# orhosko/tiny-ntt

Measured on AMD Instinct MI355X. Metric: negacyclic poly-mults/sec (n=4096, 60-bit q), bit-exact vs cg_ntt.py, higher is better.
Workload: dtype u64; 1 GPU; n=4096, q=2^60-2^14+1 (60-bit), global batch 65536 = 65536 rows on this GPU, LCG-seeded rows resident in HBM (BASELINE configs[2]); n=4096, q=1152921504606830593, rows_per_gpu=65536, global_batch=65536, variant=fused, kernel=polymul_fused_kernel, lazy_reduction=True, lib_build_id=05922c9b9694243b, parallelism=batch-sharded x1, no data-path collective

## Files before the change

### __graft_entry__.py

```python
import ctypes
import os
import subprocess
import sys

ROOT = os.path.dirname(os.path.abspath(__file__))
REFERENCE = os.environ.get("TINY_NTT_REFERENCE", "/root/reference")


def _make(directory, *targets):
    cmd = ["make", f"-j{min(8, os.cpu_count() or 1)}", "-C", os.path.join(ROOT, directory), *targets]
    r = subprocess.run(cmd, stdout=subprocess.PIPE, stderr=subprocess.STDOUT, text=True)
    if r.returncode != 0:
        sys.stderr.write(r.stdout)
        raise RuntimeError(f"build failed: {' '.join(cmd)}")


def build() -> None:
    _make("tiny_ntt_amd/csrc")
    _make("oracle", "all")
    _make("tests/emu")
    _make("tests/emu", "-f", "Makefile.prepared")
    _make("tests/emu", "-f", "Makefile.dot")
    _make("tests/devprobe")
    if os.path.isdir(os.path.join(REFERENCE, "software_benchmark")):
        _make("oracle", "ref", f"REFERENCE={REFERENCE}")
    sys.path.insert(0, ROOT)
    import tiny_ntt_amd
    from tiny_ntt_amd import engine
    lib = engine.load_library()
    missing = [s for s in engine.EXPORTED_SYMBOLS if not hasattr(lib, s)]
    if missing:
        raise RuntimeError(f"libtinyntt.so lacks symbols: {missing}")


def smoke() -> None:
    sys.path.insert(0, ROOT)
    import numpy as np
    from tiny_ntt_amd import engine

    n, q, psi = 4096, 1152921504606830593, 431606828070683274
    plan = engine.Plan(n, q, psi, device=0)
    rng = np.random.default_rng(7)
    batch = 4
    a = rng.integers(0, q, size=(batch, n), dtype=np.uint64)
    b = rng.integers(0, q, size=(batch, n), dtype=np.uint64)
    a[0, :] = q - 1
    c = plan.poly_mult(a, b)
    c_cg = plan.poly_mult(a, b, variant="cg8")

    so = os.path.join(ROOT, "oracle", "_build", "liboracle.so")
    if not os.path.exists(so):
        _make("oracle", "all")
    orc = ctypes.CDLL(so)
    P = ctypes.POINTER(ctypes.c_uint64)
    orc.tn_oracle_nwc_poly_mult_batch.argtypes = [P, P, P, ctypes.c_size_t, ctypes.c_size_t, ctypes.c_uint64, ctypes.c_uint64]
    ref = np.empty_like(a)
    rc = orc.tn_oracle_nwc_poly_mult_batch(a.ctypes.data_as(P), b.ctypes.data_as(P), ref.ctypes.data_as(P), batch, n, q, psi)
    assert rc == 0
    assert np.array_equal(c, ref), "fused kernel differs from the oracle"
    assert np.array_equal(c_cg, ref), "cg8 kernel differs from the oracle"
    print(f"smoke ok: n={n} q={q} batch={batch} fused(lazy={plan.is_lazy}) and cg8 bit-exact vs oracle")


if __name__ == "__main__":
    build()
    if len(sys.argv) > 1 and sys.argv[1] == "smoke":
        smoke()
```

### tiny_ntt_amd/csrc/fused_core.h

```cpp
#pragma once
#include <type_traits>
#include "modarith.h"

#ifndef TN_ABL_UNIFORM_TW
#define TN_ABL_UNIFORM_TW 0
#endif

namespace tn {

template <int B, int E_, typename F> struct StaticFor {
  TN_HD static void run(F& f) { f(std::integral_constant<int, B>()); StaticFor<B + 1, E_, F>::run(f); }
};
template <int E_, typename F> struct StaticFor<E_, E_, F> { TN_HD static void run(F&) {} };
template <int B, int E_, typename F> TN_HD void static_for(F&& f) { StaticFor<B, E_, F>::run(f); }

#ifndef TN_FUSED_LPT10
#define TN_FUSED_LPT10 3
#endif
#ifndef TN_FUSED_LPT12
#define TN_FUSED_LPT12 3
#endif
constexpr int fused_lpt(int logn) {
  return logn == 8 ? 2 : logn == 9 ? 3 : logn == 10 ? TN_FUSED_LPT10 : logn == 11 ? 3 : logn == 12 ? TN_FUSED_LPT12 : logn == 13 ? 3 : 0;
}
// ... 221 lines not shown
    d.pw_fold_b = d.fout > PW_IN;
    for (int r = 0; r < R; r += 2) {
      if (!BC) { b[r] = b[r + 1] = PW_OUT; continue; }
      long a0 = b[r], a1 = b[r + 1];
      if (a0 > BC_AMAX) { d.bcfold[r] = true; a0 = FOLDED; }
      if (a1 > BC_AMAX) { d.bcfold[r + 1] = true; a1 = FOLDED; }
      b[r] = tmax(a0) + tmax(tmax(a1));
      b[r + 1] = tmax(a0) + tmax(a1);
    }
    for (int g = BC ? 1 : 0; g < LOGN; ++g) {
      const int s = LOGN - 1 - g;
      if (g > 0 && phase_of(s) != phase_of(s + 1)) {
        long m = 0;
        for (int r = 0; r < R; ++r) m = b[r] > m ? b[r] : m;
        for (int r = 0; r < R; ++r) b[r] = m;
      }
      const int bit = 1 << bpos_of(s);
      for (int r = 0; r < R; ++r) {
        if (r & bit) continue;
        const int v = r | bit;
        for (int it = 0; it < 2; ++it) {
          if (b[r] + ki(b[v]) * U <= CAP && b[r] + b[v] <= CAP) break;
          if (b[r] >= b[v]) { d.ifold[g][r] = true; b[r] = FOLDED; }
          else { d.ifold[g][v] = true; b[v] = FOLDED; }
        }
        const int Kv = ki(b[v]);
        d.ik[g][r] = (unsigned char)Kv;
        const long bd = b[r] + Kv * U;
        b[r] = b[r] + b[v];
        b[v] = tmax(bd);
      }
    }
    return d;
  }
  static constexpr Data D = build();
};

template <typename Pol, typename Cfg, bool BC = false> struct SchedOf {
  typedef Sched<Pol, Cfg::LOGN> S;
  static constexpr bool fwd_fold(int s, int r) { return S::fwd_fold(s) && !(r & (1 << SplitSched<Cfg>::bpos_of(s))); }
  static constexpr int fwd_k(int, int) { return Pol::TMUL; }
  static constexpr bool inv_fold(int g, int) { return S::inv_fold(g); }
  static constexpr int inv_k(int g, int) { return S::inv_bnd(g); }
  static constexpr bool pw_fold_b() { return false; }
  static constexpr bool pw_ok() { return !Pol::lazy || S::fwd_out() <= Pol::LIMIT - 2; }
};
template <typename Cfg, bool CIN, bool BC> struct SchedOf<Policy<u64, true, CIN>, Cfg, BC> {
  typedef SplitSched<Cfg, CIN, BC> S;
  static constexpr bool fwd_fold(int s, int r) { return S::D.ffold[s][r]; }
  static constexpr int fwd_k(int s, int r) { return S::D.fk[s][r]; }
  static constexpr bool inv_fold(int g, int r) { return S::D.ifold[g][r]; }
  static constexpr int inv_k(int g, int r) { return S::D.ik[g][r]; }
  static constexpr bool pw_fold_b() { return S::D.pw_fold_b; }
  static constexpr bool pw_ok() { return true; }
  static constexpr bool bc_fold(int r) { return S::D.bcfold[r]; }
};

template <typename E> struct TwRefs {
  typedef typename TwOf<E>::type Tw;
  const Tw* __restrict__ glob;
  const Tw* lds;
  Tw* pre;
  const Tw* mid = nullptr;
  u32 zero = 0;
};

template <typename E, typename Cfg, int PH, int S_>
TN_HD typename TwOf<E>::type tw_get(const TwRefs<E>& t, u32 thi, int g) {
  constexpr int bpos = (Cfg::LOGN - 1 - S_) - Cfg::pos(PH);
  if (Cfg::tw_src(PH) == Cfg::TW_REGS) return t.pre[Cfg::pre_off(S_) + g];
  const u32 idx = (1u << S_) + (TN_ABL_UNIFORM_TW ? 0u : (thi << (Cfg::LPT - bpos - 1))) + (u32)g;
  if (Cfg::tw_src(PH) == Cfg::TW_LDS) {
    if (t.mid) return t.mid[(1 << (S_ - Cfg::stage_begin(PH))) - 1 + g];
    return t.lds[idx - Cfg::lds_tw_lo()];
  }
  if (Cfg::tw_src(PH) == Cfg::TW_VEC && t.mid) return t.mid[(1 << (S_ - Cfg::stage_begin(PH))) - 1 + g];
  return t.glob[idx + t.zero];
}

template <typename E, typename Cfg, int PH>
TN_HD void tw_fetch_vec(typename TwOf<E>::type (&mid)[Cfg::R], u32 tau, const typename TwOf<E>::type* __restrict__ glob) {
  const u32 thi = Cfg::thi(PH, tau);
  static_for<Cfg::stage_begin(PH), Cfg::stage_end(PH)>([&](auto s_) {
    constexpr int s = decltype(s_)::value;
    constexpr int bpos = (Cfg::LOGN - 1 - s) - Cfg::pos(PH);
    constexpr int cnt = Cfg::R >> (bpos + 1), off = (1 << (s - Cfg::stage_begin(PH))) - 1;
    const u32 boff = ((1u << s) + (thi << (Cfg::LPT - bpos - 1))) * (u32)sizeof(typename TwOf<E>::type);
    const typename TwOf<E>::type* base = reinterpret_cast<const typename TwOf<E>::type*>(reinterpret_cast<const char*>(glob) + boff);
#pragma unroll
    for (int g = 0; g < cnt; ++g) mid[off + g] = base[g];
  });
}

template <typename E, typename Cfg, int PH>
TN_HD void tw_fetch_mid(typename TwOf<E>::type (&mid)[Cfg::R], u32 tau, const typename TwOf<E>::type* lds_tw) {
  const u32 thi = Cfg::thi(PH, tau);
  static_for<Cfg::stage_begin(PH), Cfg::stage_end(PH)>([&](auto s_) {
    constexpr int s = decltype(s_)::value;
    constexpr int bpos = (Cfg::LOGN - 1 - s) - Cfg::pos(PH);
    constexpr int cnt = Cfg::R >> (bpos + 1), off = (1 << (s - Cfg::stage_begin(PH))) - 1;
#pragma unroll
    for (int g = 0; g < cnt; ++g)
      mid[off + g] = lds_tw[(1u << s) + (thi << (Cfg::LPT - bpos - 1)) + (u32)g - Cfg::lds_tw_lo()];
  });
}

template <typename E, typename Cfg, int S0, int S1>
TN_HD void tw_prefetch_stages(typename TwOf<E>::type* pre, u32 tau, const typename TwOf<E>::type* __restrict__ glob) {
  constexpr int PH = Cfg::PHASES - 1;
  if (Cfg::tw_src(PH) != Cfg::TW_REGS) return;
  const u32 thi = Cfg::thi(PH, tau);
  static_for<S0, S1>([&](auto s_) {
    constexpr int s = decltype(s_)::value;
    constexpr int bpos = (Cfg::LOGN - 1 - s) - Cfg::pos(PH);
    const u32 off = ((1u << s) + (thi << (Cfg::LPT - bpos - 1))) * (u32)sizeof(typename TwOf<E>::type);
    const typename TwOf<E>::type* base = reinterpret_cast<const typename TwOf<E>::type*>(reinterpret_cast<const char*>(glob) + off);
#pragma unroll
    for (int g = 0; g < Cfg::pre_count(s); ++g) pre[Cfg::pre_off(s) + g] = base[g];
  });
}
template <typename E, typename Cfg>
TN_HD void tw_prefetch_raw(typename TwOf<E>::type* pre, u32 tau, const typename TwOf<E>::type* __restrict__ glob) {
  tw_prefetch_stages<E, Cfg, Cfg::stage_begin(Cfg::PHASES - 1), Cfg::LOGN>(pre, tau, glob);
}

template <typename E, typename Cfg>
TN_HD void tw_prefetch(typename TwOf<E>::type (&pre)[Cfg::NPRE], u32 tau, const typename TwOf<E>::type* __restrict__ glob) {
  tw_prefetch_raw<E, Cfg>(pre, tau, glob);
}

template <typename E, typename Cfg, typename Pol, int PH, bool BC = false>
TN_HD void fwd_phase(E (&x)[Cfg::R], u32 tau, const TwRefs<E>& tw, const Arith<E>& ar) {
  typedef SchedOf<Pol, Cfg, BC> SO;
  typedef typename TwOf<E>::type Tw;
  const u32 thi = Cfg::thi(PH, tau);
  constexpr int SEND = BC && Cfg::stage_end(PH) == Cfg::LOGN ? Cfg::LOGN - 1 : Cfg::stage_end(PH);
  static_for<Cfg::stage_begin(PH), SEND>([&](auto s_) {
    constexpr int s = decltype(s_)::value;
    constexpr int bpos = (Cfg::LOGN - 1 - s) - Cfg::pos(PH);
    static_for<0, Cfg::R>([&](auto r_) {
      constexpr int r = decltype(r_)::value;
      if constexpr (Pol::lazy && SO::fwd_fold(s, r)) x[r] = fold(x[r], ar.k, ar.fold_c);
    });
    static_for<0, Cfg::R>([&](auto r_) {
      constexpr int r = decltype(r_)::value;
      if constexpr (!(r & (1 << bpos))) {
        const Tw w = tw_get<E, Cfg, PH, s>(tw, thi, r >> (bpos + 1));
        Pol::template ct<SO::fwd_k(s, r)>(x[r], x[r | (1 << bpos)], w, ar);
      }
    });
  });
}

template <typename E, typename Cfg, typename Pol, int PH, bool BC = false>
TN_HD void inv_phase(E (&x)[Cfg::R], u32 tau, const TwRefs<E>& tw, const Arith<E>& ar) {
  typedef SchedOf<Pol, Cfg, BC> SO;
  typedef typename TwOf<E>::type Tw;
  const u32 thi = Cfg::thi(PH, tau);
  constexpr int SEND = BC && Cfg::stage_end(PH) == Cfg::LOGN ? Cfg::LOGN - 1 : Cfg::stage_end(PH);
  static_for<0, SEND - Cfg::stage_begin(PH)>([&](auto i_) {
    constexpr int s = SEND - 1 - decltype(i_)::value;
    constexpr int g = Cfg::LOGN - 1 - s;
    constexpr int bpos = (Cfg::LOGN - 1 - s) - Cfg::pos(PH);
    static_for<0, Cfg::R>([&](auto r_) {
      constexpr int r = decltype(r_)::value;
      if constexpr (Pol::lazy && SO::inv_fold(g, r)) x[r] = fold(x[r], ar.k, ar.fold_c);
    });
    static_for<0, Cfg::R>([&](auto r_) {
      constexpr int r = decltype(r_)::value;
      if constexpr (!(r & (1 << bpos))) {
        constexpr int BND = SO::inv_k(g, r);
        if constexpr (s == 0) Pol::template gs_last<BND>(x[r], x[r | (1 << bpos)], ar);
        else {
          const Tw w = tw_get<E, Cfg, PH, s>(tw, thi, r >> (bpos + 1));
          Pol::template gs<BND>(x[r], x[r | (1 << bpos)], w, ar);
        }
      }
    });
  });
}

template <typename E, typename Cfg, typename Pol>
TN_HD void load_reduce(E (&x)[Cfg::R], const Arith<E>& ar) {
#pragma unroll
  for (int r = 0; r < Cfg::R / 2; ++r) x[r] = Pol::load(x[r], ar);
}

template <typename E, typename Cfg, int EX, int PH>
TN_HD void ex_store(const E (&x)[Cfg::R], u32 tau, E* lds) {
  E* base = lds + Cfg::ex_base(EX, PH, tau);
  static_for<0, Cfg::R>([&](auto r_) { constexpr int r = decltype(r_)::value; base[Cfg::ex_off(EX, PH, r)] = x[r]; });
}
template <typename E, typename Cfg, int EX, int PH>
TN_HD void ex_load(E (&x)[Cfg::R], u32 tau, const E* lds) {
  const E* base = lds + Cfg::ex_base(EX, PH, tau);
  static_for<0, Cfg::R>([&](auto r_) { constexpr int r = decltype(r_)::value; x[r] = base[Cfg::ex_off(EX, PH, r)]; });
}

TN_HD u64 pointwise_lazy(u64 a, u64 b, const Arith<u64>& ar) {
  return mulmod_solinas_lazy(fold(a, ar.k, ar.fold_c), b, ar.k, ar.fold_c);
}
TN_HD u32 pointwise_lazy(u32 a, u32 b, const Arith<u32>& ar) {
  return mulmod_barrett_lazy(fold(a, ar.k, ar.fold_c), fold(b, ar.k, ar.fold_c), ar.q, ar.mu, ar.k);
}
template <typename E, typename Cfg, typename Pol>
TN_HD void pointwise(E (&xa)[Cfg::R], const E (&xb)[Cfg::R], const Arith<E>& ar) {
  typedef SchedOf<Pol, Cfg> SO;
  static_assert(SO::pw_ok(), "pointwise_lazy: unfolded operand bound");
#pragma unroll
  for (int r = 0; r < Cfg::R; ++r) {
    if (Pol::lazy)
      xa[r] = pointwise_lazy(xa[r], SO::pw_fold_b() ? fold(xb[r], ar.k, ar.fold_c) : xb[r], ar);
    else
      xa[r] = mulmod_barrett(xa[r], xb[r], ar.q, ar.mu, ar.k);
    if (r & 1) sched_fence();
  }
}

TN_HD void basecase_pair(u64& a0, u64& a1, u64 b0, u64 b1, Tw64 zeta, const Arith<u64>& ar) {
  const Tw64 B0 = split_rec(b0, ar.k, ar.fold_c, ar.q), B1 = split_rec(b1, ar.k, ar.fold_c, ar.q);
  const u64 t = opaque64(mul_sp(a1, zeta, ar.sk));
  const u64 c0 = mul_sp_acc(opaque64(mul_sp(a0, B0, ar.sk)), t, B1, ar.sk);
  const u64 c1 = mul_sp_acc(opaque64(mul_sp(a0, B1, ar.sk)), a1, B0, ar.sk);
  a0 = c0;
  a1 = c1;
}
template <typename Cfg, typename Pol>
TN_HD void basecase(u64 (&xa)[Cfg::R], const u64 (&xb)[Cfg::R], const Tw64* zeta, const Arith<u64>& ar) {
  typedef SchedOf<Pol, Cfg, true> SO;
  static_assert(Pol::split && Cfg::pos(Cfg::PHASES - 1) == 0, "base case: split policy, pairs in neighbouring registers");
  static_for<0, Cfg::R / 2>([&](auto i_) {
    constexpr int r = 2 * decltype(i_)::value;
    if constexpr (SO::bc_fold(r)) xa[r] = fold(xa[r], ar.k, ar.fold_c);
    if constexpr (SO::bc_fold(r + 1)) xa[r + 1] = fold(xa[r + 1], ar.k, ar.fold_c);
    basecase_pair(xa[r], xa[r + 1], xb[r], xb[r + 1], zeta[r / 2], ar);
    sched_fence();
  });
}

template <typename E, typename Pol>
TN_HD E dot_accumulate_one(E acc, E x, const Arith<E>& ar) {
  return csub((E)(acc + Pol::canon(x, ar)), ar.q);
}
template <typename E, typename Cfg, typename Pol>
TN_HD void dot_accumulate(E (&acc)[Cfg::R], const E (&x)[Cfg::R], const Arith<E>& ar) {
#pragma unroll
  for (int r = 0; r < Cfg::R; ++r) acc[r] = dot_accumulate_one<E, Pol>(acc[r], x[r], ar);
}

}
```

### tiny_ntt_amd/csrc/kernels.hip

```cpp
#include <hip/hip_runtime.h>
#include "plan.h"
#include "dev_addr.h"

#ifndef TN_ABL_NO_BARRIER
#define TN_ABL_NO_BARRIER 0
#endif
#ifndef TN_ABL_ROWMASK
#define TN_ABL_ROWMASK 0
#endif
#ifndef TN_ABL_NO_GLOBAL
#define TN_ABL_NO_GLOBAL 0
#endif
#ifndef TN_STORE_AT_TOP
#define TN_STORE_AT_TOP 1
#endif
#ifndef TN_NT_STREAM
#define TN_NT_STREAM 1
#endif
#ifndef TN_FUSED_MIN_WAVES
#define TN_FUSED_MIN_WAVES 4
#endif
#ifndef TN_POLYMUL60_WAVES
#define TN_POLYMUL60_WAVES 6
#endif

#ifndef TN_NTTF_PIN_LOGN
#define TN_NTTF_PIN_LOGN 99
#endif
#ifndef TN_VEC_PREFETCH
#define TN_VEC_PREFETCH 1
#endif
#ifndef TN_FUSED_CIN
#define TN_FUSED_CIN 0
#endif
#ifndef TN_SADDR
#define TN_SADDR 1
#endif
#ifndef TN_KARG_ARITH
#define TN_KARG_ARITH 1
#endif
#ifndef TN_RESIDENT_TW
#define TN_RESIDENT_TW 1
#endif
#ifndef TN_SHARE_MID_TW
#define TN_SHARE_MID_TW 1
#endif
#ifndef TN_SHARE_LAST_TW
#define TN_SHARE_LAST_TW 1
#endif
#ifdef TN_MARKS
#define TN_MARK(n) asm volatile("; TNMARK " n)
#else
#define TN_MARK(n)
#endif
#ifndef TN_KERNELS_PART
#define TN_KERNELS_MAIN 1
#define TN_KERNELS_PREPARED 1
#else
#define TN_KERNELS_MAIN (TN_KERNELS_PART == 0)
#define TN_KERNELS_PREPARED (TN_KERNELS_PART == 1)
#endif
namespace tn {

#ifndef TN_SHUFFLE_LAST
#define TN_SHUFFLE_LAST 0
#endif
template <int DIST> __device__ __forceinline__ u32 lane_xor(u32 v) {
  if constexpr (DIST == 1) return (u32)__builtin_amdgcn_update_dpp(0, (int)v, 0xB1, 0xf, 0xf, false);
  else if constexpr (DIST == 2) return (u32)__builtin_amdgcn_update_dpp(0, (int)v, 0x4E, 0xf, 0xf, false);
  else {
    int r = __builtin_amdgcn_update_dpp(0, (int)v, 0x104, 0xf, 0x5, false);
    return (u32)__builtin_amdgcn_update_dpp(r, (int)v, 0x114, 0xf, 0xA, false);
  }
}
template <typename E>
__device__ __forceinline__ void transpose8_lanes(E (&x)[8], u32 lane) {
  static_for<0, 3>([&](auto b_) {
    constexpr int b = decltype(b_)::value, m = 1 << b;
    const bool hi = (lane >> b) & 1u;
    static_for<0, 8>([&](auto r_) {
      constexpr int r0 = decltype(r_)::value;
      if constexpr (!(r0 & m)) {
        constexpr int r1 = r0 | m;
        const E send = hi ? x[r0] : x[r1];
        E recv;
        if constexpr (sizeof(E) == 8) recv = ((u64)lane_xor<m>((u32)(send >> 32)) << 32) | lane_xor<m>((u32)send);
        else recv = lane_xor<m>((u32)send);
        x[r0] = hi ? recv : x[r0];
        x[r1] = hi ? x[r1] : recv;
      }
    });
  });
}

template <typename E, typename Cfg, int EX, int FROM, int TO>
__device__ __forceinline__ void exchange(E (&x)[Cfg::R], u32 tau, E* lds) {
  if constexpr (TN_SHUFFLE_LAST && Cfg::LPT == 3 && EX == Cfg::PHASES - 2 && Cfg::pos(EX + 1) == 0 && Cfg::pos(EX) == Cfg::LPT) {
    transpose8_lanes<E>(x, tau);
  } else if constexpr (Cfg::ex_wave_local(EX)) {
    __builtin_amdgcn_wave_barrier();
    ex_store<E, Cfg, EX, FROM>(x, tau, lds);
    __builtin_amdgcn_wave_barrier();
    ex_load<E, Cfg, EX, TO>(x, tau, lds);
    __builtin_amdgcn_wave_barrier();
  } else {
#if TN_ABL_NO_BARRIER
    __builtin_amdgcn_wave_barrier();
    ex_store<E, Cfg, EX, FROM>(x, tau, lds);
    __builtin_amdgcn_wave_barrier();
    ex_load<E, Cfg, EX, TO>(x, tau, lds);
    __builtin_amdgcn_wave_barrier();
#else
    __syncthreads();
    ex_store<E, Cfg, EX, FROM>(x, tau, lds);
    __syncthreads();
    ex_load<E, Cfg, EX, TO>(x, tau, lds);
    __syncthreads();
#endif
  }
}

template <typename E>
__device__ __forceinline__ const Arith<E>& kernarg_arith(u32 zero) {
  typedef const __attribute__((address_space(4))) char* KP;
  return *(const Arith<E>*)((KP)__builtin_amdgcn_kernarg_segment_ptr() + zero);
}

template <typename E, typename Cfg, typename Pol, int P0, int P1, bool KARG = false, int PRE_END = Cfg::LOGN, bool BC = false>
__device__ __forceinline__ void forward_range(E (&x)[Cfg::R], u32 tau, const TwRefs<E>& tw_in, const Arith<E>& ar_in, E* lds, bool fetch_pre,
                                              u32 tau_g) {
  typename TwOf<E>::type vec[Cfg::R];
  static_for<P0, P1>([&](auto p_) {
    constexpr int p = decltype(p_)::value;
    constexpr bool FULL = Cfg::stage_end(p) - Cfg::stage_begin(p) == Cfg::LPT;
    TN_MARK("fwd_phase");
    TwRefs<E> tw = tw_in;
    if constexpr (KARG) tw.zero = opaque_zero();
    if constexpr (TN_VEC_PREFETCH && Cfg::tw_src(p) == Cfg::TW_VEC && FULL && p > P0) tw.mid = vec;
    const Arith<E>& ar = KARG ? kernarg_arith<E>(tw.zero) : ar_in;
    fwd_phase<E, Cfg, Pol, p, BC>(x, tau, tw, ar);
    TN_MARK("fwd_other");
    if constexpr (p == Cfg::PHASES - 2) {
      if (fetch_pre) {
        sched_fence();
        tw_prefetch_stages<E, Cfg, Cfg::stage_begin(Cfg::PHASES - 1), PRE_END>(tw.pre, tau_g, tw.glob);
        sched_fence();
      }
    }
    if constexpr (p + 1 < P1) {
      constexpr int pn = p + 1 < Cfg::PHASES ? p + 1 : p;
      if constexpr (TN_VEC_PREFETCH && Cfg::tw_src(pn) == Cfg::TW_VEC && Cfg::stage_end(pn) - Cfg::stage_begin(pn) == Cfg::LPT) {
        sched_fence();
        tw_fetch_vec<E, Cfg, pn>(vec, tau_g, tw.glob);
        sched_fence();
      }
    }
    if constexpr (p + 1 < Cfg::PHASES) exchange<E, Cfg, p, p, p + 1>(x, tau, lds);
  });
}
template <typename E, typename Cfg, typename Pol>
__device__ __forceinline__ void forward_all(E (&x)[Cfg::R], u32 tau, const typename TwOf<E>::type* __restrict__ glob,
                                            const typename TwOf<E>::type* lds_tw, const Arith<E>& ar, E* lds, u32 zero = 0) {
  typename TwOf<E>::type pre[Cfg::NPRE];
  const TwRefs<E> tw = {glob, lds_tw, pre, nullptr, zero};
  forward_range<E, Cfg, Pol, 0, Cfg::PHASES>(x, tau, tw, ar, lds, true, tau);
}

template <typename E, typename Cfg, typename Pol, bool KARG = false, bool BC = false, typename F>
__device__ __forceinline__ void inverse_all(E (&x)[Cfg::R], u32 tau, const TwRefs<E>& tw_in, const Arith<E>& ar_in, E* lds,
                                            F&& after_first) {
  typename TwOf<E>::type vec[Cfg::R];
  static_for<0, Cfg::PHASES>([&](auto i_) {
    constexpr int p = Cfg::PHASES - 1 - decltype(i_)::value;
    constexpr bool FULL = Cfg::stage_end(p) - Cfg::stage_begin(p) == Cfg::LPT;
    TN_MARK("inv_phase");
    TwRefs<E> tw = tw_in;
    if constexpr (KARG) tw.zero = opaque_zero();
    if constexpr (TN_VEC_PREFETCH && Cfg::tw_src(p) == Cfg::TW_VEC && FULL && p < Cfg::PHASES - 1) tw.mid = vec;
    const Arith<E>& ar = KARG ? kernarg_arith<E>(tw.zero) : ar_in;
    inv_phase<E, Cfg, Pol, p, BC>(x, tau, tw, ar);
    TN_MARK("inv_other");
    if constexpr (p > 0) {
      constexpr int pn = p > 0 ? p - 1 : 0;
      if constexpr (TN_VEC_PREFETCH && Cfg::tw_src(pn) == Cfg::TW_VEC && Cfg::stage_end(pn) - Cfg::stage_begin(pn) == Cfg::LPT) {
        sched_fence();
        tw_fetch_vec<E, Cfg, pn>(vec, tau, tw.glob);
        sched_fence();
      }
    }
    if constexpr (p == Cfg::PHASES - 1) { sched_fence(); after_first(); sched_fence(); }
    if constexpr (p > 0) exchange<E, Cfg, p - 1, p, p - 1>(x, tau, lds);
  });
}

template <typename E> struct alignas(2 * sizeof(E)) PairOf { E lo, hi; };

#if defined(TN_FUSED_STAMPS) && TN_KERNELS_MAIN
__device__ unsigned long long tn_fused_stamps[4 * 4096];
#endif

template <typename E, typename Cfg>
__device__ __forceinline__ E ld_operand(const E* __restrict__ p, u32 row, u32 tau, int r) {
#if TN_ABL_NO_GLOBAL
  return (E)(tau * 2654435761u + 7 * r + row);
#else
#if TN_ABL_ROWMASK
  row &= TN_ABL_ROWMASK;
#endif
#if TN_NT_STREAM
  const TN_GLOBAL_AS E* rp = uniform_ptr(p + ((size_t)row << Cfg::LOGN) + Cfg::jidx(0, 0, r));
  return __builtin_nontemporal_load(rp + (Cfg::jidx(0, tau, 0) & (u32)(Cfg::N - 1)));
#else
  return p[((size_t)row << Cfg::LOGN) + Cfg::jidx(0, tau, r)];
#endif
#endif
}

template <typename E, typename Cfg>
__device__ __forceinline__ void st_result(E* __restrict__ c, u32 row, u32 tau, const E (&x)[Cfg::R]) {
#if TN_ABL_ROWMASK
  row &= TN_ABL_ROWMASK;
#endif
  const size_t off = (size_t)row << Cfg::LOGN;
#pragma unroll
  for (int r = 0; r < Cfg::R; ++r) {
#if TN_NT_STREAM
    __builtin_nontemporal_store(x[r], uniform_ptr(c + off + Cfg::jidx(0, 0, r)) + (Cfg::jidx(0, tau, 0) & (u32)(Cfg::N - 1)));
#else
    c[off + Cfg::jidx(0, tau, r)] = x[r];
#endif
  }
}

template <typename E, int LOGN, int LPT, bool LAZY>
constexpr int polymul_waves() {
  return LPT >= 4 ? 2 : (sizeof(E) == 8 && LOGN == 12 && LAZY) ? TN_POLYMUL60_WAVES : TN_FUSED_MIN_WAVES;
}

#if TN_KERNELS_MAIN
template <typename E, int LOGN, int LPT, bool LAZY, bool CIN = false, bool BC = false>
__global__ void __launch_bounds__((1 << (LOGN - LPT)), (polymul_waves<E, LOGN, LPT, LAZY>()))
polymul_fused_kernel(const Arith<E> ar, const typename TwOf<E>::type* __restrict__ tab_fwd,
                     const typename TwOf<E>::type* __restrict__ tab_inv, const E* __restrict__ a, const E* __restrict__ b,
                     E* __restrict__ c, u32 batch, u32* sched, u32 chunk) {
  typedef FusedCfg<E, LOGN, LPT> Cfg;
  typedef Policy<E, LAZY, CIN> Pol;
  extern __shared__ __attribute__((aligned(16))) unsigned char tn_smem[];
  E* lds = reinterpret_cast<E*>(tn_smem);
  typedef typename TwOf<E>::type Tw;
  const u32 tau = threadIdx.x;
  Tw* lds_fwd = reinterpret_cast<Tw*>(lds + Cfg::lds_elems());
  Tw* lds_inv = lds_fwd + Cfg::lds_tw_count();
  u32* lds_next = reinterpret_cast<u32*>(lds_inv + Cfg::lds_tw_count());
  for (u32 i = tau; i < (u32)Cfg::lds_tw_count(); i += Cfg::THREADS) {
    lds_fwd[i] = tab_fwd[Cfg::lds_tw_lo() + i];
    lds_inv[i] = tab_inv[Cfg::lds_tw_lo() + i];
  }
  __syncthreads();
  E xa[Cfg::R], xb[Cfg::R];
#ifdef TN_FUSED_STAMPS
  const unsigned long long st_t0 = __builtin_amdgcn_s_memtime(), st_r0 = __builtin_amdgcn_s_memrealtime();
#endif
  u32 row = blockIdx.x * chunk;
  u32 taken = 1;
  u32 chunk_id = blockIdx.x;
  if (row < batch) {
#pragma unroll
    for (int r = 0; r < Cfg::R; ++r) xb[r] = ld_operand<E, Cfg>(a, row, tau, r);
  }
  constexpr int PRE_END = (TN_RESIDENT_TW && polymul_waves<E, LOGN, LPT, LAZY>() <= 4 && Cfg::stage_end(Cfg::PHASES - 1) - Cfg::stage_begin(Cfg::PHASES - 1) >= 2) ? Cfg::LOGN - 1 : Cfg::LOGN;
  Tw prf[Cfg::NPRE];
  tw_prefetch_stages<E, Cfg, PRE_END, Cfg::LOGN>(prf, tau, tab_fwd);
  u32 prev = row;
  bool have_c = false;
#pragma unroll
  for (int r = 0; r < Cfg::R; ++r) xa[r] = 0;
  while (row < batch) {
    const u32 zero = opaque_zero();
    const u32 tl = opaque_copy(tau);
    const bool in_chunk = taken != chunk;
    taken = in_chunk ? taken + 1 : 1;
    chunk_id = in_chunk ? chunk_id : chunk_id + gridDim.x;
    if (tau == 0) *lds_next = in_chunk ? row + 1 : (sched ? gridDim.x + atomicAdd(&sched[0], 1u) : chunk_id) * chunk;
    TN_MARK("loop_top");
    E xn[Cfg::R];
#pragma unroll
    for (int r = 0; r < Cfg::R; ++r) xn[r] = xb[r];
    load_reduce<E, Cfg, Pol>(xn, ar);
    sched_fence();
#if TN_STORE_AT_TOP
    st_result<E, Cfg>(c, prev, tl, xa);
#endif
#pragma unroll
    for (int r = 0; r < Cfg::R; ++r) xb[r] = ld_operand<E, Cfg>(b, row, tl, r);
    sched_fence();
#pragma unroll
    for (int r = 0; r < Cfg::R; ++r) xa[r] = xn[r];
    constexpr bool KARG = TN_KARG_ARITH != 0;
    constexpr bool SHARE = TN_SHARE_LAST_TW && Cfg::PHASES >= 2;
    constexpr int PM = Cfg::PHASES >= 3 ? Cfg::PHASES - 2 : 0;
    constexpr bool SHARE2 = SHARE && TN_SHARE_MID_TW && Cfg::PHASES >= 3 && Cfg::tw_src(PM) == Cfg::TW_LDS &&
                            Cfg::stage_end(PM) - Cfg::stage_begin(PM) == Cfg::LPT;
    const TwRefs<E> twf = {tab_fwd, lds_fwd, prf, nullptr, zero};
    static_assert(!BC || SHARE2, "base case: built for the shared-twiddle schedule only");
    if constexpr (SHARE2) forward_range<E, Cfg, Pol, 0, PM, KARG, Cfg::LOGN, BC>(xa, tau, twf, ar, lds, false, tl);
    else if constexpr (SHARE) forward_range<E, Cfg, Pol, 0, Cfg::PHASES - 1, KARG>(xa, tau, twf, ar, lds, false, tl);
    else forward_all<E, Cfg, Pol>(xa, tau, tab_fwd, lds_fwd, ar, lds, zero);
    __syncthreads();
    const u32 next = wave_uniform(*lds_next);
    load_reduce<E, Cfg, Pol>(xb, ar);
    if constexpr (SHARE2) {
      forward_range<E, Cfg, Pol, 0, PM, KARG, Cfg::LOGN, BC>(xb, tau, twf, ar, lds, false, tl);
      Tw mid[Cfg::R];
      tw_fetch_mid<E, Cfg, PM>(mid, tau, lds_fwd);
      const TwRefs<E> twm = {tab_fwd, lds_fwd, prf, mid, zero};
      forward_range<E, Cfg, Pol, PM, PM + 1, KARG, Cfg::LOGN, BC>(xa, tau, twm, ar, lds, false, tl);
      forward_range<E, Cfg, Pol, PM, PM + 1, KARG, PRE_END, BC>(xb, tau, twm, ar, lds, true, tl);
      forward_range<E, Cfg, Pol, PM + 1, Cfg::PHASES, KARG, Cfg::LOGN, BC>(xb, tau, twf, ar, lds, false, tl);
      forward_range<E, Cfg, Pol, PM + 1, Cfg::PHASES, KARG, Cfg::LOGN, BC>(xa, tau, twf, ar, lds, false, tl);
    } else if constexpr (SHARE) {
      forward_range<E, Cfg, Pol, 0, Cfg::PHASES - 1, KARG, PRE_END>(xb, tau, twf, ar, lds, true, tl);
      forward_range<E, Cfg, Pol, Cfg::PHASES - 1, Cfg::PHASES, KARG>(xb, tau, twf, ar, lds, false, tl);
      forward_range<E, Cfg, Pol, Cfg::PHASES - 1, Cfg::PHASES, KARG>(xa, tau, twf, ar, lds, false, tl);
    } else {
      forward_all<E, Cfg, Pol>(xb, tau, tab_fwd, lds_fwd, ar, lds, zero);
    }
    Tw pre[Cfg::NPRE];
    if constexpr (BC) {
      TN_MARK("basecase");
      basecase<Cfg, Pol>(xa, xb, prf + Cfg::pre_off(Cfg::LOGN - 1), ar);
      sched_fence();
      tw_prefetch_stages<E, Cfg, Cfg::stage_begin(Cfg::PHASES - 1), Cfg::LOGN - 1>(pre, tl, tab_inv);
    } else {
      tw_prefetch<E, Cfg>(pre, tl, tab_inv);
      TN_MARK("pointwise");
      pointwise<E, Cfg, Pol>(xa, xb, ar);
    }
    TN_MARK("after_pointwise");
    const TwRefs<E> twi = {tab_inv, lds_inv, pre, nullptr, zero};
    inverse_all<E, Cfg, Pol, KARG, BC>(xa, tau, twi, ar, lds, [&]() {
      const u32 nrow = next < batch ? next : row;
#pragma unroll
      for (int r = 0; r < Cfg::R; ++r) xb[r] = ld_operand<E, Cfg>(a, nrow, tl, r);
    });
#if TN_STORE_AT_TOP
    prev = row;
    have_c = true;
#else
    st_result<E, Cfg>(c, row, tau, xa);
#endif
    row = next;
  }
  if (have_c) st_result<E, Cfg>(c, prev, tau, xa);
#ifdef TN_FUSED_STAMPS
  if (tau == 0 && blockIdx.x < 4096) {
    tn_fused_stamps[4 * blockIdx.x + 0] = st_t0; tn_fused_stamps[4 * blockIdx.x + 1] = st_r0;
    tn_fused_stamps[4 * blockIdx.x + 2] = __builtin_amdgcn_s_memtime(); tn_fused_stamps[4 * blockIdx.x + 3] = __builtin_amdgcn_s_memrealtime();
  }
#endif
  if (sched && tau == 0 && atomicAdd(&sched[1], 1u) == gridDim.x - 1) { sched[0] = 0; sched[1] = 0; }
}

template <typename E, int LOGN, int LPT, bool LAZY, int MODE>
__global__ void __launch_bounds__((1 << (LOGN - LPT)), (LPT >= 4 ? 2 : TN_FUSED_MIN_WAVES))
ntt_fused_kernel(const Arith<E> ar, const typename TwOf<E>::type* __restrict__ tab, const E* __restrict__ in, E* __restrict__ out, u32 batch,
                 u32* sched, u32 chunk) {
  typedef FusedCfg<E, LOGN, LPT> Cfg;
  typedef Policy<E, LAZY> Pol;
  typedef typename TwOf<E>::type Tw;
  extern __shared__ __attribute__((aligned(16))) unsigned char tn_smem[];
  E* lds = reinterpret_cast<E*>(tn_smem);
  const u32 tau = threadIdx.x;
  E* nat = lds + Cfg::lds_elems();
  Tw* lds_tab = reinterpret_cast<Tw*>(nat + Cfg::N);
  u32* lds_next = reinterpret_cast<u32*>(lds_tab + Cfg::lds_tw_count());
  for (u32 i = tau; i < (u32)Cfg::lds_tw_count(); i += Cfg::THREADS) lds_tab[i] = tab[Cfg::lds_tw_lo() + i];
  u32 left = chunk - 1, chunk_id = blockIdx.x;
  auto take_next = [&](u32 cur, u32 slot) {
    if (left) { --left; lds_next[slot] = cur + 1; }
    else {
      chunk_id = sched ? gridDim.x + atomicAdd(&sched[0], 1u) : chunk_id + gridDim.x;
      left = chunk - 1;
      lds_next[slot] = chunk_id * chunk;
    }
  };
  if (tau == 0) take_next(blockIdx.x * chunk, 1u);
  __syncthreads();
  u32 next = wave_uniform(lds_next[1]);
  constexpr int LAST = Cfg::PHASES - 1;
  E xn[Cfg::R];
  u32 row = blockIdx.x * chunk;
  if (row < batch) {
#pragma unroll
    for (int r = 0; r < Cfg::R; ++r) xn[r] = ld_operand<E, Cfg>(in, row, tau, r);
  }
  for (u32 it = 0; row < batch; ++it) {
    if (tau == 0) take_next(next, it & 1u);
    constexpr bool PIN = LOGN >= TN_NTTF_PIN_LOGN;
    const u32 zero = PIN ? opaque_zero() : 0u;
    const u32 tl = PIN ? opaque_copy(tau) : tau;
    constexpr bool KARG = PIN && TN_KARG_ARITH != 0;
    E x[Cfg::R];
#pragma unroll
    for (int r = 0; r < Cfg::R; ++r) x[r] = xn[r];
    sched_fence();
    if (MODE != FNTT_CYCLIC_INV && next < batch) {
#pragma unroll
      for (int r = 0; r < Cfg::R; ++r) xn[r] = ld_operand<E, Cfg>(in, next, tl, r);
    }
    sched_fence();
    if (MODE == FNTT_CYCLIC_INV) {
#pragma unroll
      for (int r = 0; r < Cfg::R; ++r) x[r] = Pol::load(x[r], ar);
#pragma unroll
      for (int r = 0; r < Cfg::R; ++r) nat[Cfg::nat_addr(Cfg::jidx(0, tau, r))] = x[r];
      __syncthreads();
#pragma unroll
      for (int r = 0; r < Cfg::R; ++r) x[r] = nat[Cfg::nat_addr(bitrev(Cfg::jidx(LAST, tau, r), LOGN))];
      Tw pre[Cfg::NPRE];
      tw_prefetch<E, Cfg>(pre, tl, tab);
      const TwRefs<E> tw = {tab, lds_tab, pre, nullptr, zero};
      inverse_all<E, Cfg, Pol, KARG>(x, tau, tw, ar, lds, [&]() {
        if (next < batch) {
#pragma unroll
          for (int r = 0; r < Cfg::R; ++r) xn[r] = ld_operand<E, Cfg>(in, next, tl, r);
        }
      });
      st_result<E, Cfg>(out, row, tl, x);
    } else {
#pragma unroll
      for (int r = 0; r < Cfg::R / 2; ++r) x[r] = Pol::load(x[r], ar);
      if (!LAZY) {
#pragma unroll
        for (int r = Cfg::R / 2; r < Cfg::R; ++r) x[r] = Pol::load(x[r], ar);
      }
      {
        Tw pre[Cfg::NPRE];
        const TwRefs<E> tw = {tab, lds_tab, pre, nullptr, zero};
        forward_range<E, Cfg, Pol, 0, Cfg::PHASES, KARG>(x, tau, tw, ar, lds, true, tl);
      }
#pragma unroll
      for (int r = 0; r < Cfg::R; ++r)
        nat[Cfg::nat_addr(bitrev(Cfg::jidx(LAST, tau, r), LOGN))] = LAZY ? Pol::canon(x[r], ar) : x[r];
      __syncthreads();
#pragma unroll
      for (int r = 0; r < Cfg::R; ++r) x[r] = nat[Cfg::nat_addr(Cfg::jidx(0, tau, r))];
      st_result<E, Cfg>(out, row, tl, x);
    }
    if (Cfg::THREADS <= 64) __syncthreads();
    row = next;
    next = wave_uniform(lds_next[it & 1u]);
  }
  if (sched && tau == 0 && atomicAdd(&sched[1], 1u) == gridDim.x - 1) { sched[0] = 0; sched[1] = 0; }
}

template <typename E, int LOGN, int LPT, bool LAZY>
static hipError_t launch_nttf_t(const tn_plan* p, int mode, const void* in, void* out, size_t batch, hipStream_t s) {
  typedef FusedCfg<E, LOGN, LPT> Cfg;
  typedef typename TwOf<E>::type Tw;
  const size_t lds_bytes = (size_t)(Cfg::lds_elems() + Cfg::N) * sizeof(E) + (size_t)Cfg::lds_tw_count() * sizeof(Tw) + 16;
  const PlanView<E> pv = make_view<E>(p);
  auto kern = ntt_fused_kernel<E, LOGN, LPT, LAZY, FNTT_TWIST_FWD>;
  if (mode == FNTT_CYCLIC_FWD) kern = ntt_fused_kernel<E, LOGN, LPT, LAZY, FNTT_CYCLIC_FWD>;
  else if (mode != FNTT_TWIST_FWD) kern = ntt_fused_kernel<E, LOGN, LPT, LAZY, FNTT_CYCLIC_INV>;
  const FusedNttSetup<E> su = fused_ntt_setup(pv.ar, mode);
  return launch_persistent(p, s, (const void*)kern, Cfg::THREADS, lds_bytes, Cfg::N * sizeof(E), batch, FUSED_ROWS, [&](u32 grid, u32* sched, u32 chunk) {
    const Tw* tab = fused_table(pv, su.tab);
    const E* in_ = (const E*)in; E* out_ = (E*)out; u32 b32 = (u32)batch;
    Arith<E> ar = su.ar;
    void* args[] = {&ar, &tab, &in_, &out_, &b32, &sched, &chunk};
    return hipLaunchKernel((const void*)kern, dim3(grid), dim3(Cfg::THREADS), args, lds_bytes, s);
  });
}

template <typename E, bool LAZY>
static hipError_t launch_nttf_e(const tn_plan* p, int mode, const void* in, void* out, size_t batch, hipStream_t s) {
#ifdef TN_ONLY_MAIN
  return hipErrorInvalidValue;
#else
  switch (p->logn) {
    case 8: return launch_nttf_t<E, 8, fused_lpt(8), LAZY>(p, mode, in, out, batch, s);
    case 9: return launch_nttf_t<E, 9, fused_lpt(9), LAZY>(p, mode, in, out, batch, s);
    case 10: return launch_nttf_t<E, 10, fused_lpt(10), LAZY>(p, mode, in, out, batch, s);
    case 11: return launch_nttf_t<E, 11, fused_lpt(11), LAZY>(p, mode, in, out, batch, s);
    case 12: return launch_nttf_t<E, 12, fused_lpt(12), LAZY>(p, mode, in, out, batch, s);
    case 13: return launch_nttf_t<E, 13, fused_lpt(13), LAZY>(p, mode, in, out, batch, s);
    default: return hipErrorInvalidValue;
  }
#endif
}

hipError_t launch_ntt_fused(const tn_plan* p, int mode, const void* in, void* out, size_t batch, hipStream_t s) {
  if (batch == 0) return hipSuccess;
  if (p->elem_bytes == 8)
    return p->lazy ? launch_nttf_e<u64, true>(p, mode, in, out, batch, s) : launch_nttf_e<u64, false>(p, mode, in, out, batch, s);
  return p->lazy ? launch_nttf_e<u32, true>(p, mode, in, out, batch, s) : launch_nttf_e<u32, false>(p, mode, in, out, batch, s);
}
// ... 606 lines not shown
```

Measured before the change: 30.50 million poly-mults/s.

## Keep basecase twiddles resident and pair mid-phase forward butterflies with streamed LDS twiddles

For the lazy 60-bit n=4096 basecase kernel, the last-stage forward twiddles stay resident in registers (pinned with opaque moves) instead of being refetched each row. The middle forward phase for both operands now runs through a new paired routine that streams LDS twiddle records one at a time and applies each to both polynomials, replacing the shared 'mid' register array. The read of the next row index is moved after pointwise, and inverse LDS phases use a separate tau index. The goal is to cut twiddle reloads and register pressure at 6 waves, but it risks spills and a different instruction schedule.

New measurement: 30.72 million poly-mults/s (median of 6 runs). No clear change (+0.7%).

```diff
diff --git a/__graft_entry__.py b/__graft_entry__.py
--- a/__graft_entry__.py
+++ b/__graft_entry__.py
@@ -21,6 +21,7 @@
     _make("tests/emu")
     _make("tests/emu", "-f", "Makefile.prepared")
     _make("tests/emu", "-f", "Makefile.dot")
+    _make("tests/emu", "-f", "Makefile.resident")
     _make("tests/devprobe")
     if os.path.isdir(os.path.join(REFERENCE, "software_benchmark")):
         _make("oracle", "ref", f"REFERENCE={REFERENCE}")
diff --git a/tiny_ntt_amd/csrc/fused_core.h b/tiny_ntt_amd/csrc/fused_core.h
--- a/tiny_ntt_amd/csrc/fused_core.h
+++ b/tiny_ntt_amd/csrc/fused_core.h
@@ -397,6 +397,40 @@
   });
 }
 
+constexpr int pair_rec_stage(int i) { int j = 0; while ((2 << j) <= i + 1) ++j; return j; }
+template <typename E, typename Cfg, typename Pol, int PH, bool BC = false>
+TN_HD void fwd_phase_pair(E (&xa)[Cfg::R], E (&xb)[Cfg::R], u32 tau, const typename TwOf<E>::type* lds_tw, const Arith<E>& ar) {
+  typedef SchedOf<Pol, Cfg, BC> SO;
+  typedef typename TwOf<E>::type Tw;
+  static_assert(Cfg::tw_src(PH) == Cfg::TW_LDS && Cfg::stage_end(PH) - Cfg::stage_begin(PH) == Cfg::LPT, "a full LDS-sourced phase");
+  const u32 thi = Cfg::thi(PH, tau);
+  auto rec = [&](auto i_) -> Tw {
+    constexpr int i = decltype(i_)::value, j = pair_rec_stage(i), s = Cfg::stage_begin(PH) + j, g = i + 1 - (1 << j);
+    constexpr int bpos = (Cfg::LOGN - 1 - s) - Cfg::pos(PH);
+    return lds_tw[(1u << s) + (thi << (Cfg::LPT - bpos - 1)) + (u32)g - Cfg::lds_tw_lo()];
+  };
+  Tw wn = rec(std::integral_constant<int, 0>{});
+  static_for<0, Cfg::R - 1>([&](auto i_) {
+    constexpr int i = decltype(i_)::value, j = pair_rec_stage(i), s = Cfg::stage_begin(PH) + j, g = i + 1 - (1 << j);
+    constexpr int bpos = (Cfg::LOGN - 1 - s) - Cfg::pos(PH);
+    const Tw w = wn;
+    if constexpr (i + 1 < Cfg::R - 1) wn = rec(std::integral_constant<int, i + 1>{});
+    auto side = [&](E (&x)[Cfg::R]) {
+      static_for<0, Cfg::R>([&](auto r_) {
+        constexpr int r = decltype(r_)::value;
+        if constexpr (Pol::lazy && g == 0 && SO::fwd_fold(s, r)) x[r] = fold(x[r], ar.k, ar.fold_c);
+      });
+      static_for<0, Cfg::R>([&](auto r_) {
+        constexpr int r = decltype(r_)::value;
+        if constexpr (!(r & (1 << bpos)) && (r >> (bpos + 1)) == g) Pol::template ct<SO::fwd_k(s, r)>(x[r], x[r | (1 << bpos)], w, ar);
+      });
+    };
+    side(xa);
+    side(xb);
+    sched_fence();
+  });
+}
+
 template <typename E, typename Cfg, typename Pol, int PH, bool BC = false>
 TN_HD void inv_phase(E (&x)[Cfg::R], u32 tau, const TwRefs<E>& tw, const Arith<E>& ar) {
   typedef SchedOf<Pol, Cfg, BC> SO;
diff --git a/tiny_ntt_amd/csrc/kernels.hip b/tiny_ntt_amd/csrc/kernels.hip
--- a/tiny_ntt_amd/csrc/kernels.hip
+++ b/tiny_ntt_amd/csrc/kernels.hip
@@ -41,6 +41,9 @@
 #endif
 #ifndef TN_RESIDENT_TW
 #define TN_RESIDENT_TW 1
+#endif
+#ifndef TN_RESIDENT_BC_TW
+#define TN_RESIDENT_BC_TW 1
 #endif
 #ifndef TN_SHARE_MID_TW
 #define TN_SHARE_MID_TW 1
@@ -168,7 +171,7 @@
 
 template <typename E, typename Cfg, typename Pol, bool KARG = false, bool BC = false, typename F>
 __device__ __forceinline__ void inverse_all(E (&x)[Cfg::R], u32 tau, const TwRefs<E>& tw_in, const Arith<E>& ar_in, E* lds,
-                                            F&& after_first) {
+                                            F&& after_first, u32 tau_tw) {
   typename TwOf<E>::type vec[Cfg::R];
   static_for<0, Cfg::PHASES>([&](auto i_) {
     constexpr int p = Cfg::PHASES - 1 - decltype(i_)::value;
@@ -178,7 +181,7 @@
     if constexpr (KARG) tw.zero = opaque_zero();
     if constexpr (TN_VEC_PREFETCH && Cfg::tw_src(p) == Cfg::TW_VEC && FULL && p < Cfg::PHASES - 1) tw.mid = vec;
     const Arith<E>& ar = KARG ? kernarg_arith<E>(tw.zero) : ar_in;
-    inv_phase<E, Cfg, Pol, p, BC>(x, tau, tw, ar);
+    inv_phase<E, Cfg, Pol, p, BC>(x, Cfg::tw_src(p) == Cfg::TW_LDS ? tau_tw : tau, tw, ar);
     TN_MARK("inv_other");
     if constexpr (p > 0) {
       constexpr int pn = p > 0 ? p - 1 : 0;
@@ -192,8 +195,19 @@
     if constexpr (p > 0) exchange<E, Cfg, p - 1, p, p - 1>(x, tau, lds);
   });
 }
+template <typename E, typename Cfg, typename Pol, bool KARG = false, bool BC = false, typename F>
+__device__ __forceinline__ void inverse_all(E (&x)[Cfg::R], u32 tau, const TwRefs<E>& tw_in, const Arith<E>& ar_in, E* lds,
+                                            F&& after_first) {
+  inverse_all<E, Cfg, Pol, KARG, BC>(x, tau, tw_in, ar_in, lds, after_first, tau);
+}
 
 template <typename E> struct alignas(2 * sizeof(E)) PairOf { E lo, hi; };
+
+template <typename E, int N>
+__device__ __forceinline__ void pin_records(typename TwOf<E>::type* rec) {
+#pragma unroll
+  for (int i = 0; i < N; ++i) { rec[i].w = opaque64(rec[i].w); rec[i].wp = opaque64(rec[i].wp); }
+}
 
 #if defined(TN_FUSED_STAMPS) && TN_KERNELS_MAIN
 __device__ unsigned long long tn_fused_stamps[4 * 4096];
@@ -236,6 +250,9 @@
 constexpr int polymul_waves() {
   return LPT >= 4 ? 2 : (sizeof(E) == 8 && LOGN == 12 && LAZY) ? TN_POLYMUL60_WAVES : TN_FUSED_MIN_WAVES;
 }
+
+template <typename E, int LOGN, int LPT, bool LAZY, bool BC>
+constexpr bool resident_bc_tw() { return TN_RESIDENT_TW && TN_RESIDENT_BC_TW && BC && sizeof(E) == 8 && LOGN == 12 && LPT == 3 && LAZY; }
 
 #if TN_KERNELS_MAIN
 template <typename E, int LOGN, int LPT, bool LAZY, bool CIN = false, bool BC = false>
@@ -268,7 +285,8 @@
 #pragma unroll
     for (int r = 0; r < Cfg::R; ++r) xb[r] = ld_operand<E, Cfg>(a, row, tau, r);
   }
-  constexpr int PRE_END = (TN_RESIDENT_TW && polymul_waves<E, LOGN, LPT, LAZY>() <= 4 && Cfg::stage_end(Cfg::PHASES - 1) - Cfg::stage_begin(Cfg::PHASES - 1) >= 2) ? Cfg::LOGN - 1 : Cfg::LOGN;
+  constexpr bool RES_BC = resident_bc_tw<E, LOGN, LPT, LAZY, BC>();
+  constexpr int PRE_END = (TN_RESIDENT_TW && (polymul_waves<E, LOGN, LPT, LAZY>() <= 4 || RES_BC) && Cfg::stage_end(Cfg::PHASES - 1) - Cfg::stage_begin(Cfg::PHASES - 1) >= 2) ? Cfg::LOGN - 1 : Cfg::LOGN;
   Tw prf[Cfg::NPRE];
   tw_prefetch_stages<E, Cfg, PRE_END, Cfg::LOGN>(prf, tau, tab_fwd);
   u32 prev = row;
@@ -282,6 +300,7 @@
     taken = in_chunk ? taken + 1 : 1;
     chunk_id = in_chunk ? chunk_id : chunk_id + gridDim.x;
     if (tau == 0) *lds_next = in_chunk ? row + 1 : (sched ? gridDim.x + atomicAdd(&sched[0], 1u) : chunk_id) * chunk;
+    if constexpr (RES_BC) pin_records<E, Cfg::pre_count(Cfg::LOGN - 1)>(prf + Cfg::pre_off(Cfg::LOGN - 1));
     TN_MARK("loop_top");
     E xn[Cfg::R];
 #pragma unroll
@@ -307,9 +326,22 @@
     else if constexpr (SHARE) forward_range<E, Cfg, Pol, 0, Cfg::PHASES - 1, KARG>(xa, tau, twf, ar, lds, false, tl);
     else forward_all<E, Cfg, Pol>(xa, tau, tab_fwd, lds_fwd, ar, lds, zero);
     __syncthreads();
-    const u32 next = wave_uniform(*lds_next);
+    u32 next = 0;
+    if constexpr (!RES_BC) next = wave_uniform(*lds_next);
     load_reduce<E, Cfg, Pol>(xb, ar);
-    if constexpr (SHARE2) {
+    if constexpr (RES_BC) {
+      forward_range<E, Cfg, Pol, 0, PM, KARG, Cfg::LOGN, BC>(xb, tau, twf, ar, lds, false, tl);
+      TN_MARK("fwd_pair");
+      fwd_phase_pair<E, Cfg, Pol, PM, BC>(xa, xb, tau, lds_fwd, KARG ? kernarg_arith<E>(opaque_zero()) : ar);
+      TN_MARK("fwd_other");
+      sched_fence();
+      tw_prefetch_stages<E, Cfg, Cfg::stage_begin(Cfg::PHASES - 1), PRE_END>(prf, tl, tab_fwd);
+      sched_fence();
+      exchange<E, Cfg, PM, PM, PM + 1>(xa, tau, lds);
+      exchange<E, Cfg, PM, PM, PM + 1>(xb, tau, lds);
+      forward_range<E, Cfg, Pol, PM + 1, Cfg::PHASES, KARG, Cfg::LOGN, BC>(xb, tau, twf, ar, lds, false, tl);
+      forward_range<E, Cfg, Pol, PM + 1, Cfg::PHASES, KARG, Cfg::LOGN, BC>(xa, tau, twf, ar, lds, false, tl);
+    } else if constexpr (SHARE2) {
       forward_range<E, Cfg, Pol, 0, PM, KARG, Cfg::LOGN, BC>(xb, tau, twf, ar, lds, false, tl);
       Tw mid[Cfg::R];
       tw_fetch_mid<E, Cfg, PM>(mid, tau, lds_fwd);
@@ -337,12 +369,13 @@
       pointwise<E, Cfg, Pol>(xa, xb, ar);
     }
     TN_MARK("after_pointwise");
+    if constexpr (RES_BC) next = wave_uniform(*lds_next);
     const TwRefs<E> twi = {tab_inv, lds_inv, pre, nullptr, zero};
     inverse_all<E, Cfg, Pol, KARG, BC>(xa, tau, twi, ar, lds, [&]() {
       const u32 nrow = next < batch ? next : row;
 #pragma unroll
       for (int r = 0; r < Cfg::R; ++r) xb[r] = ld_operand<E, Cfg>(a, nrow, tl, r);
-    });
+    }, RES_BC ? tl : tau);
 #if TN_STORE_AT_TOP
     prev = row;
     have_c = true;
```
